# DaehwanKimLab/centrifuge

Measured on NVIDIA H100. Metric: reads/sec (100 bp SE classification), higher is better.
Workload: dtype u64

## Files before the change

centrifuge_b200/csrc/cf_logic.h:

```cpp
#ifndef CF_LOGIC_H_
#define CF_LOGIC_H_

#include <stdint.h>

#ifdef __CUDACC__
#define CFB_HD __host__ __device__ __forceinline__
#define CFB_HDN __host__ __device__
#else
#define CFB_HD inline
#define CFB_HDN inline
#endif

namespace cfb {

static const uint64_t kOff = 0xffffffffffffffffull;
static const uint64_t kUnk = 0xfffffffffffffffeull;
static const uint32_t kBwNone = 0xffffffffu;

struct IndexView {
	const uint64_t* sides;
	const uint64_t* ftab;
	const uint64_t* eftab;
	const uint16_t* sample16;
	const uint32_t* sample32;
	const uint64_t* brow;
	const uint32_t* bseq;
	const uint32_t* bbits;
	const uint64_t* seq_taxid;
	const int32_t*  seq_path;
	const uint64_t* paths;
	const uint8_t*  seq_excluded;
	const uint64_t* host_taxids;
	const uint64_t* rank16;
	const uint64_t* ftab2;
	const uint16_t* rtab16;
	const uint32_t* rtab32;
	const uint64_t* ftabk;
	const uint64_t* walk8;
	uint64_t walk8_rows;
	int32_t  ftabd_chars;
	uint64_t len, zoff, zside, fchr[4], last_boundary, num_sides;
	uint32_t zoffc, n_boundaries, n_seqs, n_host;
	int32_t  off_rate, ftab_chars, bshift, ftabk_chars;
};

struct Params {
	uint32_t khits, min_hitlen, ihits, increment;
	uint32_t tree_traverse, class_rank_slot;
};

struct HitRec { uint64_t top, bot; uint32_t bwoff, len; };

static const uint64_t kRowMask = (1ull << 40) - 1ull, kRowStart = 1ull << 63, kRowSameTs = 1ull << 58;

struct Counters {
	unsigned long long units, partial_searches, ftab_probes, sides_search, walk_steps, rows_resolved, lf_steps, ext_searches;
	unsigned long long req_rank16, req_ftab2, req_ftabk, req_walk8, req_ftabd;
};

CFB_HD int popc64(uint64_t x) {
#ifdef __CUDA_ARCH__
	return __popcll(x);
#else
	return __builtin_popcountll(x);
#endif
}

CFB_HD uint64_t match2(uint64_t w, int c) {
	uint64_t y = ~(w ^ ((uint64_t)c * 0x5555555555555555ull));
	return y & (y >> 1) & 0x5555555555555555ull;
}

CFB_HD int bwt_char(const IndexView& v, uint64_t row) {
#ifdef __CUDA_ARCH__
	if(v.rank16) {
		const uint64_t* e = v.rank16 + (row >> 6) * 8;
		const uint32_t o = (uint32_t)(row & 63);
		return (int)(((e[3] >> o) & 1ull) * 1 + ((e[5] >> o) & 1ull) * 2 + ((e[7] >> o) & 1ull) * 3);
	}
#endif
	uint64_t s = row / 384; uint32_t off = (uint32_t)(row - s * 384);
	return (int)((v.sides[s * 16 + (off >> 5)] >> ((off & 31) * 2)) & 3);
}

CFB_HD uint64_t lf_scalar(const IndexView& v, uint64_t row, int c) {
#ifdef __CUDA_ARCH__
	if(v.rank16) {
		const uint64_t* e = v.rank16 + ((row >> 6) * 4 + (uint64_t)c) * 2;
		return v.fchr[c] + (e[0] & 0x7fffffffffffffffull) + (uint64_t)popc64(e[1] & (((uint64_t)1 << (row & 63)) - 1));
	}
#endif
	uint64_t s = row / 384; uint32_t off = (uint32_t)(row - s * 384);
	const uint64_t* w = v.sides + s * 16;
	uint32_t full = off >> 5, rem = off & 31;
	uint64_t n = 0;
	for(uint32_t k = 0; k < full; k++) n += (uint64_t)popc64(match2(w[k], c));
	if(rem) n += (uint64_t)popc64(match2(w[full], c) & (((uint64_t)1 << (2 * rem)) - 1));
	if(c == 0 && s == v.zside && v.zoffc < off) n--;
	return v.fchr[c] + w[12 + c] + n;
}

CFB_HD int seq_at(const uint8_t* fw, uint32_t len, int strand, uint32_t j) {
	if(strand == 0) return fw[j];
	int c = fw[len - 1 - j];
	return c > 3 ? 4 : 3 - c;
}

CFB_HD uint64_t ftab_hi(const IndexView& v, uint64_t e) { return e <= v.len ? e : v.eftab[(e ^ kOff) * 2 + 1]; }
CFB_HD uint64_t ftab_lo(const IndexView& v, uint64_t e) { return e <= v.len ? e : v.eftab[(e ^ kOff) * 2]; }

// ... 479 lines not shown
```

centrifuge_b200/csrc/cfb200.cu:

```cuda
#include "../../include/cfb200.h"
#include "cf_index.h"
#include "cf_kernels.cuh"

#include <algorithm>
#include <atomic>
#include <mutex>
#include <thread>
#include <fcntl.h>
#include <unistd.h>
#include <cstdarg>
#include <cstdio>
#include <cstring>
#include <set>
#include <string>
#include <vector>

using namespace cfb;

enum { M_DONE = 0, M_FTAB = 1, M_LF = 2, M_NEED = 3, M_FTABK = 4 };

struct SearchArgs {
	IndexView v; Params p; BatchView b;
	HitRec* hits; uint32_t* nhits; uint32_t cap;
	unsigned long long* task_ctr64; uint32_t ntasks, chunk;
// ... 179 lines not shown
		}
		y = 0;
		for(int e = 0; e < 64; e++) if(dv[e] == 0) y |= 1ull << e;
		for(uint32_t e = 0; e < 64; e++) if(ftabk_death(y, e) != dv[e]) { y = ~0ull; break; }
	}
	const uint64_t w = bot - top;
	out[fk] = make_ulonglong2(top | ((w < kFtabkWide ? w : kFtabkWide) << 40), y);
}

template <int RW> struct ReadRegs {
	uint64_t rw[RW]; uint32_t nw[RW];
	__device__ __forceinline__ void load(const uint64_t* pk, const uint32_t* nm, uint32_t W) {
		#pragma unroll
		for(int k = 0; k < RW; k++) { rw[k] = (uint32_t)k < W ? __ldg(pk + k) : 0ull; nw[k] = (uint32_t)k < W ? __ldg(nm + k) : 0u; }
	}
	__device__ __forceinline__ uint64_t word(uint32_t k) const {
		uint64_t v = 0;
		#pragma unroll
		for(int q = 0; q < RW; q++) if((uint32_t)q == k) v = rw[q];
		return v;
	}
	__device__ __forceinline__ uint32_t nword(uint32_t k) const {
		uint32_t v = 0;
		#pragma unroll
		for(int q = 0; q < RW; q++) if((uint32_t)q == k) v = nw[q];
		return v;
	}
	__device__ __forceinline__ int base(uint32_t p) const {
		const uint32_t k = p >> 5, sh = p & 31;
		return ((nword(k) >> sh) & 1u) ? 4 : (int)((word(k) >> (2 * sh)) & 3);
	}
	__device__ __forceinline__ void window(uint32_t p, uint64_t& win, uint32_t& nwin) const {
		const uint32_t k = p >> 5, sh = p & 31;
		win = shr64(word(k), 2 * sh) | shl64(word(k + 1), 64 - 2 * sh);
		nwin = (uint32_t)(((uint64_t)nword(k) | ((uint64_t)nword(k + 1) << 32)) >> sh);
	}
};

template <int COUNT, int RW>
__global__ void __launch_bounds__(kSearchThreads) k_search_t(const SearchArgs a) {
	const ulonglong2* r16 = reinterpret_cast<const ulonglong2*>(a.v.rank16);
	const ulonglong2* ftab2 = reinterpret_cast<const ulonglong2*>(a.v.ftab2);
	const ulonglong2* ftabk = reinterpret_cast<const ulonglong2*>(a.v.ftabk);
	const uint32_t fk = (COUNT == 1 || !a.v.ftabk) ? 0u : (uint32_t)a.v.ftabk_chars;
	const uint32_t fc = (uint32_t)a.v.ftab_chars;
	const unsigned long long* w8 = COUNT == 1 ? nullptr : reinterpret_cast<const unsigned long long*>(a.v.walk8);
	const uint32_t fd = (fk == 0 || a.p.min_hitlen < (uint32_t)a.v.ftabd_chars) ? 0u : (uint32_t)a.v.ftabd_chars;
	ReadRegs<RW> rd;
	uint64_t top = 0, bot = 0, fi = 0;
	uint32_t rlen = 0, tid = 0, cur = 0, dep = 0, offset = 0, nh = 0, nt = 0, slow_until = 0, fail_w = 0, fail_at = 0xffffffffu;
	bool nolong = true;
	int mode = M_NEED;
	unsigned long long c_ps = 0, c_ft = 0, c_sides = 0, c_lf = 0;
	unsigned long long q_r16 = 0, q_f2 = 0, q_fk = 0, q_w8 = 0;
	WarpPool pool; pool.base = pool.end = 0;
	bool more = true;

	auto emit = [&](uint64_t t, uint64_t b, uint32_t off, uint32_t len) {
		if(a.keep_short || len >= kLongLen) {
			if(nh < a.cap) { HitRec* h = a.hits + (size_t)tid * a.cap + nh; h->top = t; h->bot = b; h->bwoff = off; h->len = len; }
			else atomicExch(a.overflow, 1u);
			nh++;
		}
		nt++;
		if(len >= a.p.min_hitlen) nolong = false;
	};
	auto after_hit = [&](uint32_t hlen) -> bool {
		bool done = cur >= rlen;
		if(!done) { if(hlen > a.p.increment) cur += 1; if(cur + a.p.min_hitlen >= rlen) done = true; }
		if(done) { a.nhits[tid] = nh_pack(nh, nt, nolong); mode = M_NEED; return false; }
		return true;
	};
	auto start_search = [&]() {
		for(;;) {
			if(COUNT == 1) c_ps++;
			offset = cur;
			if(rlen - cur < fc) { emit(kOff, kOff, offset, rlen - offset); a.nhits[tid] = nh_pack(nh, nt, nolong); mode = M_NEED; return; }
			uint64_t win; uint32_t nwin; rd.window(cur, win, nwin);
			const uint32_t nbits = nwin & ((1u << fc) - 1u);
			if(nbits) {
				const uint32_t hl = (uint32_t)__ffs(nbits);
				cur += hl;
				emit(kOff, kOff, offset, hl);
				if(after_hit(hl)) continue; else return;
			}
			if(fk && rlen - cur >= fk && !(nwin & ((1u << fk) - 1u))) {
				fi = win & ((1ull << (2 * fk)) - 1ull);
				if(fd && rlen - cur >= fd && !(nwin & ((1u << fd) - 1u))) fi |= (64ull | ((win >> (2 * fk)) & 63ull)) << (2 * fk);
				mode = M_FTABK;
				return;
			}
			fi = win & ((1ull << (2 * fc)) - 1ull);
			mode = M_FTAB;
			return;
		}
	};
	auto hit_and_restart = [&]() {
		const uint32_t hl = dep - offset;
		emit(top, bot, offset, hl);
		cur = dep;
		if(after_hit(hl)) start_search();
	};

	for(;;) {
		{
			const bool want = mode == M_NEED;
			if(more) {
				unsigned long long t = 0;
				const bool got = pool_take(pool, want, a.task_ctr64, (unsigned long long)a.ntasks, a.chunk, t);
				if(want) {
					if(got) {
						tid = (uint32_t)t;
						const uint32_t per = 2u * (uint32_t)a.b.n_mates;
						const uint32_t unit = tid / per, rem = tid - unit * per;
						const int mate = (int)(rem >> 1);
						const uint8_t fl = a.b.flags ? a.b.flags[unit] : 3;
						nh = 0; nt = 0; rlen = a.b.len[mate][unit];
						if(!((fl >> mate) & 1) || rlen == 0) a.nhits[tid] = 0;
						else { rd.load(a.pk + (size_t)tid * a.W, a.nm + (size_t)tid * a.W, a.W); cur = 0; slow_until = 0; fail_w = 0; fail_at = 0xffffffffu; nolong = true; start_search(); }
					} else mode = M_DONE;
				}
				if(__any_sync(0xffffffffu, want && !got)) more = false;
			} else if(want) mode = M_DONE;
		}
		if(!__any_sync(0xffffffffu, mode != M_DONE)) break;
		int c = 4;
		const bool lf = mode == M_LF;
		bool range = false, jump = false, known_fail = false;
		const void* p0 = nullptr; const void* p1 = nullptr; uint32_t sub = 0;
		if(mode == M_FTAB) { p0 = ftab2 + fi; if(COUNT == 2) q_f2++; }
		else if(mode == M_FTABK) { p0 = ftabk + (fi & ((1ull << (2 * fk)) - 1ull)); if(COUNT == 2) q_fk++; }
		else if(lf) {
			c = rd.base(dep);
			if(c <= 3) {
				range = (bot - top) != 1;
				const uint64_t width = bot - top;
				if(dep == fail_at && !range) known_fail = true;
				else if(w8 && width <= (uint64_t)a.jump_w && (dep >= slow_until || width < (uint64_t)fail_w) && rlen - dep >= 8 && bot <= a.v.walk8_rows) {
					jump = true; p0 = w8 + (top & ~1ull); sub = (uint32_t)(top & 1); if(COUNT == 2) q_w8++;
					if(range) { const uint64_t last = bot - 1; sub |= (uint32_t)(last & 1) << 1; if((last & ~1ull) != (top & ~1ull)) { p1 = w8 + (last & ~1ull); if(COUNT == 2) q_w8++; } }
				} else {
					p0 = r16 + (top >> 6) * 4 + c;
					if(COUNT == 2) q_r16++;
					if(range && (bot >> 6) != (top >> 6)) { p1 = r16 + (bot >> 6) * 4 + c; if(COUNT == 2) q_r16++; }
				}
			}
		}
		ulonglong2 e = make_ulonglong2(0, 0), bq;
		asm volatile("{\n\t.reg .pred p;\n\tsetp.ne.u64 p, %2, 0;\n\t@p ld.global.nc.v2.u64 {%0, %1}, [%2];\n\t}" : "+l"(e.x), "+l"(e.y) : "l"(p0));
		bq = e;
		asm volatile("{\n\t.reg .pred p;\n\tsetp.ne.u64 p, %2, 0;\n\t@p ld.global.nc.v2.u64 {%0, %1}, [%2];\n\t}" : "+l"(bq.x), "+l"(bq.y) : "l"(p1));
		const ulonglong2 tq = e;
		if(mode == M_FTABK) {
			const uint32_t ext = (uint32_t)(fi >> (2 * fk));
			const uint32_t dv = ext ? ftabk_death(e.y, ext & 63u) : 0u;
			const uint64_t width = e.x >> 40;
			if(dv) {
				const uint32_t hl = fk + dv - 1u;
				emit(kUnk, kUnk, offset, hl);
				cur += hl;
				if(after_hit(hl)) start_search();
			} else if(width != 0 && width != kFtabkWide) {
				top = e.x & kRowMask; bot = top + width; dep = cur + fk;
				if(dep < rlen) mode = M_LF; else hit_and_restart();
			} else { fi &= (1ull << (2 * fc)) - 1ull; mode = M_FTAB; }
		} else if(mode == M_FTAB) {
			if(COUNT == 1) c_ft++;
			top = e.x; bot = e.y;
			dep = cur + fc;
			if(bot <= top) {
				const uint32_t hl = dep - offset;
				emit(kOff, kOff, offset, hl);
				cur = dep;
				if(after_hit(hl)) start_search();
			} else if(dep < rlen) mode = M_LF;
			else hit_and_restart();
		} else if(jump) {
			uint64_t win; uint32_t nwin; rd.window(dep, win, nwin);
			const uint64_t w = (sub & 1u) ? e.y : e.x;
			const uint64_t wl = (sub & 2u) ? bq.y : bq.x;
			const uint64_t width = bot - top;
			if((w >> 56) == 8 && !(nwin & 0xffu) && !(((w >> 40) ^ win) & 0xffffull)
			   && (width == 1 || ((wl >> 40) == (w >> 40) && (wl & kWalkRowMask) - (w & kWalkRowMask) == width - 1))) {
				top = w & kWalkRowMask; bot = top + width; dep += 8;
				if(dep >= rlen) hit_and_restart();
			} else {
				slow_until = dep + 8; fail_w = (uint32_t)width;
				if(width == 1) {
					const uint32_t diff = (uint32_t)(((w >> 40) ^ win) & 0xffffull), nb = nwin & 0xffu, nv = (uint32_t)(w >> 56) & 0xffu;
					uint32_t good = diff ? (uint32_t)(__ffs(diff) - 1) >> 1 : 8u;
					if(nb) good = min(good, (uint32_t)(__ffs(nb) - 1));
					good = min(good, nv);
					fail_at = good < 8u ? dep + good : 0xffffffffu;
				}
			}
		} else if(lf) {
			bool fail = c > 3 || known_fail;
			uint64_t t = 0, b = 0;
			if(!fail) {
				const uint32_t oT = (uint32_t)(top & 63), oB = (uint32_t)(bot & 63);
				t = a.v.fchr[c] + (tq.x & kOccMask) + (uint64_t)__popcll(tq.y & ((1ull << oT) - 1ull));
				if(range) b = a.v.fchr[c] + (bq.x & kOccMask) + (uint64_t)__popcll(bq.y & ((1ull << oB) - 1ull));
				else {
					if(!((tq.y >> oT) & 1ull)) fail = true;
					b = t + 1;
				}
				if(b <= t) fail = true;
				if(COUNT == 1) {
					uint64_t sT; uint32_t offT; row_locus(top, sT, offT);
					const bool same_side = !range || (bot - top) < (uint64_t)(384 - offT);
					c_lf += range ? 2 : 1; c_sides += same_side ? 1 : 2;
				}
			}
			if(fail) hit_and_restart();
			else { top = t; bot = b; dep++; if(dep >= rlen) hit_and_restart(); }
		}
	}
	if(COUNT == 1 && a.ctr) {
		atomicAdd(&a.ctr->partial_searches, c_ps); atomicAdd(&a.ctr->ftab_probes, c_ft);
		atomicAdd(&a.ctr->sides_search, c_sides); atomicAdd(&a.ctr->lf_steps, c_lf);
	}
	if(COUNT == 2 && a.ctr) {
		atomicAdd(&a.ctr->req_rank16, q_r16); atomicAdd(&a.ctr->req_ftab2, q_f2); atomicAdd(&a.ctr->req_ftabk, q_fk); atomicAdd(&a.ctr->req_walk8, q_w8);
	}
}

struct UnitArgs {
	IndexView v; Params p; BatchView b;
	HitRec* hits; uint32_t* nhits; uint32_t cap;
	uint32_t* nrows;
	uint64_t* row_off;
	unsigned long long* row_total;
	uint64_t* rows; uint32_t* ids; uint64_t rows_cap;
	Entry* entries; TaxCnt* tcs; OutRec* recs_sparse; uint32_t* nout;
	unsigned int* overflow;
	Counters* ctr;
	HitRec* regen; uint32_t* regen_n; unsigned long long* regen_ctr; uint64_t regen_slots; uint32_t full_cap; uint32_t keep_short;
};

__device__ uint32_t search_strand_dev(const IndexView& v, const Params& p, const uint8_t* fw, uint32_t len, int strand, HitRec* hits, uint32_t cap) {
	const ulonglong2* r16 = reinterpret_cast<const ulonglong2*>(v.rank16);
	const ulonglong2* ftab2 = reinterpret_cast<const ulonglong2*>(v.ftab2);
	const ulonglong2* ftabk = reinterpret_cast<const ulonglong2*>(v.ftabk);
	const uint32_t fc = (uint32_t)v.ftab_chars, fk = v.ftabk ? (uint32_t)v.ftabk_chars : 0u;
	auto base = [&](uint32_t d) -> int { return seq_at(fw, len, strand, len - 1 - d); };
	uint32_t cur = 0, n = 0;
	if(len == 0) return 0;
	for(;;) {
		HitRec h; h.bwoff = cur; uint32_t new_cur; bool done = false;
		const uint32_t offset = cur;
		if(len - cur < fc) { h.top = h.bot = kOff; h.len = len - offset; new_cur = len; done = true; }
		else {
			uint32_t firstn = 0xffffffffu; uint64_t fi = 0;
			const uint32_t span = (fk && len - cur >= fk) ? fk : fc;
			for(uint32_t i = 0; i < span; i++) { const int c = base(cur + i); if(c > 3) { firstn = i; break; } fi |= (uint64_t)c << (2 * i); }
			if(firstn < fc) { new_cur = cur + firstn + 1; h.top = h.bot = kOff; h.len = new_cur - offset; done = new_cur >= len; }
			else {
				uint64_t top = 0, bot = 0; uint32_t dep = 0; bool have = false;
				if(span == fk && fk > fc && firstn == 0xffffffffu) {
					const uint64_t x = __ldg(&ftabk[fi].x), width = x >> 40;
					if(width != 0 && width != kFtabkWide) { top = x & kRowMask; bot = top + width; dep = cur + fk; have = true; }
				}
				if(!have) { const ulonglong2 e = __ldg(ftab2 + (fi & ((1ull << (2 * fc)) - 1ull))); top = e.x; bot = e.y; dep = cur + fc; }
				if(bot <= top) { h.top = h.bot = kOff; h.len = dep - offset; new_cur = dep; done = dep >= len; }
				else {
					while(dep < len) {
						const int c = base(dep);
						if(c > 3) break;
						if(bot - top == 1) {
							if(v.walk8 && top < v.walk8_rows && len - dep >= 8) {
								const uint64_t e = __ldg(v.walk8 + top);
								bool ok = (e >> 56) == 8;
								for(uint32_t j = 0; ok && j < 8; j++) ok = base(dep + j) == (int)((e >> (40 + 2 * j)) & 3);
								if(ok) { top = e & kWalkRowMask; bot = top + 1; dep += 8; continue; }
							}
							const ulonglong2 e = __ldg(r16 + (top >> 6) * 4 + c);
							if(!((e.y >> (top & 63)) & 1ull)) break;
							top = v.fchr[c] + (e.x & kOccMask) + (uint64_t)__popcll(e.y & ((1ull << (top & 63)) - 1ull)); bot = top + 1; dep++;
						} else {
							const ulonglong2 et = __ldg(r16 + (top >> 6) * 4 + c);
							const ulonglong2 eb = (bot >> 6) == (top >> 6) ? et : __ldg(r16 + (bot >> 6) * 4 + c);
							const uint64_t t = v.fchr[c] + (et.x & kOccMask) + (uint64_t)__popcll(et.y & ((1ull << (top & 63)) - 1ull));
							const uint64_t b = v.fchr[c] + (eb.x & kOccMask) + (uint64_t)__popcll(eb.y & ((1ull << (bot & 63)) - 1ull));
							if(b <= t) break;
							top = t; bot = b; dep++;
						}
					}
					h.top = top; h.bot = bot; h.len = dep - offset; new_cur = dep; done = dep >= len;
				}
			}
		}
		if(n < cap) hits[n] = h;
		n++;
		cur = new_cur;
		if(done) break;
		if(h.len > p.increment) cur += 1;
		if(cur + p.min_hitlen >= len) break;
	}
	return n;
}

static const uint32_t kWindowLen = 320;
template <int COUNT>
__global__ void __launch_bounds__(kSearchThreads) k_search_long(const SearchArgs a) {
	const uint32_t per = 2u * (uint32_t)a.b.n_mates;
	Counters local; memset(&local, 0, sizeof local);
	for(uint32_t tid = blockIdx.x * blockDim.x + threadIdx.x; tid < a.ntasks; tid += gridDim.x * blockDim.x) {
		const uint32_t unit = tid / per, rem = tid - unit * per;
		const int mate = (int)(rem >> 1), strand = (int)(rem & 1);
		const uint8_t fl = a.b.flags ? a.b.flags[unit] : 3;
		const uint32_t len = a.b.len[mate][unit];
		if(!((fl >> mate) & 1) || len == 0) { a.nhits[tid] = 0; continue; }
		const uint8_t* fw = a.b.bases + a.b.off[mate][unit];
		HitRec* hits = a.hits + (size_t)tid * a.cap;
		const uint32_t n = COUNT == 1 ? search_strand_scalar(a.v, a.p, fw, len, strand, hits, a.cap, &local)
		                              : search_strand_dev(a.v, a.p, fw, len, strand, hits, a.cap);
		if(n > a.cap) atomicExch(a.overflow, 1u);
		a.nhits[tid] = nh_pack(min(n, a.cap), n, false);
	}
	if(COUNT == 1 && a.ctr) {
		atomicAdd(&a.ctr->partial_searches, local.partial_searches); atomicAdd(&a.ctr->ftab_probes, local.ftab_probes);
		atomicAdd(&a.ctr->sides_search, local.sides_search); atomicAdd(&a.ctr->lf_steps, local.lf_steps);
	}
}

typedef void (*SearchKernel)(const SearchArgs);
static SearchKernel search_kernel(uint32_t maxlen, int count) {
// ... 205 lines not shown
	uint64_t idx = 0, row = 0;
	int mode = R_NEED;
	unsigned long long c_walk = 0, c_rows = 0;
	WarpPool pool; pool.base = pool.end = 0;
	bool more = true;
	auto put = [&](uint32_t v) { if(IDENT && a.ids16) a.ids16[idx] = (uint16_t)v; else a.ids[idx] = v; };
	auto settle = [&](uint64_t r) -> int {
		if(r == a.v.zoff) { if(gl == 0) put(0); return R_NEED; }
		if((r & lowmask) == 0) return R_SAMPLE;
		return R_WALK;
	};
	for(;;) {
		{
			const bool want = mode == R_NEED;
			if(more) {
				unsigned long long t = 0;
				bool got = pool_take(pool, want && gl == 0, a.task_ctr, (unsigned long long)n, a.chunk, t);
				t = __shfl_sync(0xffffffffu, t, gbase); got = __shfl_sync(0xffffffffu, (int)got, gbase) != 0;
				if(want) {
					if(got) { idx = t; row = IDENT ? idx : (a.rows[idx] & kRowMask); if(COUNT && gl == 0) c_rows++; mode = settle(row); }
					else mode = R_DONE;
				}
				if(__any_sync(0xffffffffu, want && !got)) more = false;
			} else if(want) mode = R_DONE;
		}
		if(!__any_sync(0xffffffffu, mode != R_DONE)) break;
		ulonglong2 e = make_ulonglong2(0, 0); uint32_t samp = 0;
		if(mode == R_WALK) e = __ldg(r16 + (row >> 6) * 4 + gl);
		else if(mode == R_SAMPLE && gl == 0) samp = a.v.sample32 ? __ldg(a.v.sample32 + (row >> a.v.off_rate)) : (uint32_t)__ldg(a.v.sample16 + (row >> a.v.off_rate));
		if(mode == R_SAMPLE) { if(gl == 0) put(samp); mode = R_NEED; }
		else if(mode == R_WALK) {
			const uint32_t off = (uint32_t)(row & 63);
			const unsigned flagged = __shfl_sync(gmask, (unsigned)(e.x >> 63), gbase);
			bool found = false;
			if(flagged && a.v.last_boundary > 0 && row <= a.v.last_boundary) {
				uint32_t lo = 0, hi = a.v.n_boundaries;
				while(lo < hi) { const uint32_t mid = (lo + hi) >> 1; if(a.v.brow[mid] < row) lo = mid + 1; else hi = mid; }
				if(lo < a.v.n_boundaries && a.v.brow[lo] == row) { found = true; if(gl == 0) put(a.v.sample32 ? a.v.bseq[lo] : (uint32_t)(uint16_t)a.v.bseq[lo]); }
			}
			if(found) mode = R_NEED;
			else {
				const uint64_t mine = a.v.fchr[gl] + (e.x & kOccMask) + (uint64_t)__popcll(e.y & ((1ull << off) - 1ull));
				const unsigned who = (__ballot_sync(gmask, (e.y >> off) & 1ull) >> gbase) & 0xFu;
				const int src = __ffs(who) - 1;
				row = __shfl_sync(gmask, mine, gbase + (src < 0 ? 0 : src));
				if(COUNT && gl == 0) c_walk++;
				mode = settle(row);
			}
		}
	}
	if(COUNT && gl == 0 && a.ctr) { atomicAdd(&a.ctr->walk_steps, c_walk); atomicAdd(&a.ctr->rows_resolved, c_rows); }
}

__global__ void __launch_bounds__(kSearchThreads) k_build_walk8(IndexView v, uint64_t nrows, uint64_t* out) {
	const unsigned lane = threadIdx.x & 31, gl = lane & 3, gbase = lane & 28, gmask = 0xFu << gbase;
	const ulonglong2* r16 = reinterpret_cast<const ulonglong2*>(v.rank16);
	const uint64_t ngroups = (uint64_t)gridDim.x * (kSearchThreads / 4);
	const uint64_t per = (nrows + ngroups - 1) / ngroups;
	const uint64_t g = (uint64_t)blockIdx.x * (kSearchThreads / 4) + (threadIdx.x >> 2);
	for(uint64_t idx = g * per; idx < min(nrows, (g + 1) * per); idx++) {
		uint64_t row = idx, chars = 0; uint32_t nv = 0;
		for(; nv < 8; nv++) {
			if(row == v.zoff) break;
			const ulonglong2 e = __ldg(r16 + (row >> 6) * 4 + gl);
			const uint32_t off = (uint32_t)(row & 63);
			const uint64_t mine = v.fchr[gl] + (e.x & kOccMask) + (uint64_t)__popcll(e.y & ((1ull << off) - 1ull));
			const unsigned who = (__ballot_sync(gmask, (e.y >> off) & 1ull) >> gbase) & 0xFu;
			const int src = __ffs(who) - 1;
			if(src < 0) break;
			chars |= (uint64_t)src << (2 * nv);
			row = __shfl_sync(gmask, mine, gbase + src);
		}
		if(gl == 0) out[idx] = (row & kWalkRowMask) | (chars << 40) | ((uint64_t)nv << 56);
	}
}

__global__ void __launch_bounds__(256) k_lookup(const ResolveArgs a) {
	uint64_t n = *a.total; if(n > a.rows_cap) return;
	const uint64_t i = (uint64_t)blockIdx.x * blockDim.x + threadIdx.x;
	const uint64_t stride = (uint64_t)gridDim.x * blockDim.x;
	for(uint64_t k = i; k < n; k += stride) { const uint64_t r = a.rows[k] & kRowMask; a.ids[k] = a.v.rtab32 ? __ldg(a.v.rtab32 + r) : (uint32_t)__ldg(a.v.rtab16 + r); }
}

__global__ void __launch_bounds__(128) k_compact(uint32_t n_units, const uint64_t* row_off, const uint64_t* out_off,
                                                 const OutRec* sparse, OutRec* dense, uint32_t* rec_off32, uint64_t dense_cap, unsigned int* overflow) {
	const uint32_t unit = blockIdx.x * blockDim.x + threadIdx.x;
	if(unit > n_units) return;
	if(unit == n_units) { rec_off32[unit] = (uint32_t)out_off[unit]; return; }
	const uint64_t o = out_off[unit], n = out_off[unit + 1] - o;
	rec_off32[unit] = (uint32_t)o;
	if(o + n > dense_cap) { if(n) atomicExch(overflow, 3u); return; }
	const uint64_t src = row_off[unit];
	for(uint64_t i = 0; i < n; i++) dense[o + i] = sparse[src + i];
}

__global__ void k_test_lf(IndexView v, const uint64_t* rows, const uint8_t* chars, uint64_t n, uint64_t* out) {
	for(uint64_t i = (uint64_t)blockIdx.x * blockDim.x + threadIdx.x; i < n; i += (uint64_t)gridDim.x * blockDim.x) {
		const int c = chars[i] > 3 ? bwt_char(v, rows[i]) : chars[i];
		out[i] = lf_scalar(v, rows[i], c);
	}
}

static thread_local char g_err[512] = "";
static int fail(int code, const char* fmt, ...) {
	va_list ap; va_start(ap, fmt); vsnprintf(g_err, sizeof g_err, fmt, ap); va_end(ap); return code;
}
#define CK(call) do { cudaError_t e_ = (call); if(e_ != cudaSuccess) return fail(CFB_ECUDA, "%s failed: %s (%s:%d)", #call, cudaGetErrorString(e_), __FILE__, __LINE__); } while(0)

extern "C" const char* cfb_last_error(void) { return g_err; }
extern "C" const char* cfb_version(void) { return "cfb200 0.1 (sm_90a)"; }

template <class T> struct DBuf {
	T* p = nullptr; size_t cap = 0;
	cudaError_t ensure(size_t n) {
		if(n <= cap) return cudaSuccess;
		if(p) cudaFree(p);
		p = nullptr; cap = 0;
		size_t want = n + n / 8 + 16;
		cudaError_t e = cudaMalloc((void**)&p, want * sizeof(T));
		if(e == cudaSuccess) cap = want;
		return e;
	}
	void release() { if(p) cudaFree(p); p = nullptr; cap = 0; }
};
template <class T> struct HBuf {
	T* p = nullptr; size_t cap = 0;
// ... 106 lines not shown
			uint64_t* f2 = nullptr; const uint64_t nf = h.ftab_len - 1;
			CKX(cudaMalloc((void**)&f2, nf * 16));
			ix->dptrs.push_back(f2); ix->device_bytes += nf * 16;
			k_build_ftab2<<<(unsigned)((nf + 255) / 256), 256>>>(v, nf, f2);
			CKX(cudaDeviceSynchronize());
			v.rank16 = r16; v.ftab2 = f2;
			ix->tables.rank16_bytes = (nb + 1) * 64; ix->tables.ftab2_bytes = nf * 16;
			cudaFree((void*)v.sides);
			ix->dptrs.erase(std::find(ix->dptrs.begin(), ix->dptrs.end(), (void*)v.sides));
			ix->device_bytes -= h.num_sides * h.side_sz; v.sides = nullptr;
			size_t free_b = 0, total_b = 0; cudaMemGetInfo(&free_b, &total_b);
			double head_gb = 12.0; { const char* e = getenv("CFB_HBM_HEADROOM_GB"); if(e) head_gb = atof(e); }
			const uint64_t headroom = std::min<uint64_t>((uint64_t)(head_gb * 1073741824.0), free_b / 2);
			auto budget = [&]() -> uint64_t { size_t f = 0, t = 0; cudaMemGetInfo(&f, &t); return f > headroom ? f - headroom : 0; };
			{
				const char* ed = getenv("CFB_FTABD");
				const bool death = !(ed && ed[0] == '0');
				int K = 0;
				{ const char* e = getenv("CFB_FTABK"); if(e) K = atoi(e); else { K = h.ftab_chars; while(K < 15 && (4ull << (2 * K)) <= h.len / 4) K++; } }
				while(K > h.ftab_chars && (16ull << (2 * K)) > budget() / 2) K--;
				if(K <= h.ftab_chars || K > 16) K = death ? h.ftab_chars : 0;
				const uint64_t nk = K ? 1ull << (2 * K) : 0;
				if(K && h.len + 1 < (1ull << 40) && nk * 16 <= budget()) {
					ulonglong2* fk = nullptr;
					CKX(cudaMalloc((void**)&fk, nk * 16));
					ix->dptrs.push_back(fk); ix->device_bytes += nk * 16;
					k_build_ftabk<<<(unsigned)((nk + 127) / 128), 128>>>(v, K, nk, death, fk);
					CKX(cudaDeviceSynchronize());
					v.ftabk = (const uint64_t*)fk; v.ftabk_chars = K; v.ftabd_chars = death ? K + 3 : 0;
					ix->tables.ftabk_bytes = nk * 16; ix->tables.ftabk_chars = K; ix->tables.ftabd_chars = v.ftabd_chars;
				}
			}
			{
				const char* e = (flags & CFB_LOAD_NO_RESOLVE_TABLE) ? "0" : getenv("CFB_RESOLVE_TABLE");
				const uint64_t nrows = h.len + 1, esz = h.wide_sample ? 4 : 2;
				if(!(e && e[0] == '0') && nrows * esz + 16 <= budget()) {
					void* tab = nullptr; unsigned long long* sc = nullptr;
					CKX(cudaMalloc(&tab, nrows * esz + 16)); CKX(cudaMalloc((void**)&sc, 16));
					ix->dptrs.push_back(tab); ix->device_bytes += nrows * esz;
					const unsigned long long init[2] = {0ull, (unsigned long long)nrows};
					CKX(cudaMemcpy(sc, init, 16, cudaMemcpyHostToDevice));
					ResolveArgs ra; ra.v = v; ra.rows = nullptr; ra.ids = h.wide_sample ? (uint32_t*)tab : nullptr; ra.ids16 = h.wide_sample ? nullptr : (uint16_t*)tab;
					ra.total = (const uint64_t*)(sc + 1); ra.rows_cap = nrows; ra.task_ctr = sc; ra.chunk = 256; ra.ctr = nullptr;
					int occ = 1; cudaOccupancyMaxActiveBlocksPerMultiprocessor(&occ, k_resolve_c<false, true>, kSearchThreads, 0);
					k_resolve_c<false, true><<<prop.multiProcessorCount * std::max(occ, 1), kSearchThreads>>>(ra);
					CKX(cudaDeviceSynchronize());
					cudaFree(sc);
					if(h.wide_sample) v.rtab32 = (const uint32_t*)tab; else v.rtab16 = (const uint16_t*)tab;
					ix->tables.resolve_table_bytes = nrows * esz; ix->tables.resolve_entry_bytes = (int32_t)esz;
				}
			}
			{
				const char* e = (flags & CFB_LOAD_NO_WALK8) ? "0" : getenv("CFB_WALK8");
				const uint64_t nrows = h.len + 1;
				uint64_t cover = std::min<uint64_t>(nrows, budget() / 8);
				{ const char* f = getenv("CFB_WALK8_ROWS"); if(f) cover = std::min<uint64_t>(nrows, strtoull(f, NULL, 10)); }
				if(!(e && e[0] == '0') && nrows < (1ull << 40) && cover >= nrows / 8 && cover > 0) {
					void* tab = nullptr;
					CKX(cudaMalloc(&tab, cover * 8 + 16));
					ix->dptrs.push_back(tab); ix->device_bytes += cover * 8;
					int occ = 1; cudaOccupancyMaxActiveBlocksPerMultiprocessor(&occ, k_build_walk8, kSearchThreads, 0);
					k_build_walk8<<<prop.multiProcessorCount * std::max(occ, 1) * 4, kSearchThreads>>>(v, cover, (uint64_t*)tab);
					CKX(cudaDeviceSynchronize());
					v.walk8 = (const uint64_t*)tab; v.walk8_rows = cover;
					ix->tables.walk8_bytes = cover * 8; ix->tables.walk8_rows = cover;
				}
			}
		}
		{ size_t fb = 0, tb = 0; cudaMemGetInfo(&fb, &tb); ix->tables.total_bytes = ix->device_bytes; ix->tables.free_bytes_after_load = fb; }
		std::vector<uint8_t>().swap(ix->h.sides);
	}
	*out = ix;
	return CFB_OK;
}
#undef CKX
extern "C" int cfb_index_load(const char* basename, int device, cfb_index** out) { return cfb_index_load_ex(basename, device, 0u, out); }
extern "C" void cfb_index_free(cfb_index* ix) {
	if(!ix) return;
	if(ix->device >= 0) { cudaSetDevice(ix->device); for(size_t i = 0; i < ix->dptrs.size(); i++) cudaFree(ix->dptrs[i]); }
	delete ix;
}
extern "C" int cfb_index_get_info(const cfb_index* ix, cfb_index_info* o) {
	if(!ix || !o) return fail(CFB_EINVAL, "null argument");
	const HostIndex& h = ix->h;
	o->len = h.len; o->num_sides = h.num_sides; o->n_seqs = h.seq_taxid.size(); o->n_tax_nodes = h.nodes.size();
	o->n_boundaries = h.brow.size(); o->line_rate = h.line_rate; o->off_rate = h.off_rate; o->ftab_chars = h.ftab_chars;
	o->sample_bytes = h.wide_sample ? 4 : 2; o->compressed = h.compressed ? 1 : 0; o->device = ix->device; o->device_bytes = ix->device_bytes;
	return CFB_OK;
}
extern "C" int cfb_index_get_tables(const cfb_index* ix, cfb_index_tables* o) {
	if(!ix || !o) return fail(CFB_EINVAL, "null argument");
	*o = ix->tables;
	return CFB_OK;
}
extern "C" const char* cfb_index_seq_name(const cfb_index* ix, uint32_t s) { return (ix && s < ix->h.seq_name.size()) ? ix->h.seq_name[s].c_str() : NULL; }
extern "C" uint64_t cfb_index_seq_taxid(const cfb_index* ix, uint32_t s) { return (ix && s < ix->h.seq_taxid.size()) ? ix->h.seq_taxid[s] : 0; }
extern "C" int cfb_index_tax_node(const cfb_index* ix, uint64_t taxid, uint64_t* parent, int* rank, int* leaf) {
	const TaxNode* n = ix ? ix->h.find_node(taxid) : NULL;
	if(!n) return 0;
	if(parent) *parent = n->parent; if(rank) *rank = n->rank; if(leaf) *leaf = n->leaf;
	return 1;
}
extern "C" const cfb::HostIndex* cfb_index_host(const cfb_index* ix) { return ix ? &ix->h : NULL; }
extern "C" int cfb_index_node_taxids(const cfb_index* ix, uint64_t* out, uint64_t cap) {
	if(!ix || !out || cap < ix->h.nodes.size()) return fail(CFB_EINVAL, "cfb_index_node_taxids: buffer too small");
	for(size_t i = 0; i < ix->h.nodes.size(); i++) out[i] = ix->h.nodes[i].taxid;
	return CFB_OK;
}
extern "C" void cfb_params_default(cfb_params* p) {
	if(!p) return;
	memset(p, 0, sizeof *p); p->khits = 5; p->min_hitlen = 22; p->tree_traverse = 1; p->class_rank_slot = 0;
}

static const int kSlots = 17;

struct Slot {
	cudaStream_t st = nullptr;
	cudaEvent_t ev[6] = {nullptr, nullptr, nullptr, nullptr, nullptr, nullptr};
// ... 24 lines not shown

struct cfb_dbatch { int slot; uint64_t n_units; };
struct TextCtx;
static void text_release(cfb_ctx*);
static void comm_release(cfb_ctx*);

struct CountsCtx {
	bool ready = false;
	std::vector<uint64_t> h_taxid; DBuf<uint64_t> d_taxid; uint32_t n = 0;
	DBuf<unsigned long long> total, global; bool reduced = false;
	void release() { d_taxid.release(); total.release(); global.release(); }
};

struct cfb_ctx {
	const cfb_index* ix = nullptr;
	IndexView view; Params prm;
	DBuf<uint8_t> d_excl; DBuf<uint64_t> d_host;
	Slot slots[kSlots];
	Counters* d_ctr = nullptr; int count = 0;
	uint64_t launches = 0;
	int resolve_blocks = 0;
	cfb_dbatch resident; bool resident_used = false;
	double rec_ratio = 2.0;
	uint64_t rows_cap0 = 0;
	TextCtx* text = nullptr;
	CountsCtx cnt; bool fold_records = false;
	uint32_t jump_w = 4; bool keep_short = false;
	uint64_t regen_lists = 0, regen_tasks = 0;
	uint64_t regen_slots0 = 0;
	void* comm = nullptr; int comm_rank = 0, comm_size = 1; cudaStream_t comm_st = nullptr;
};

static void expand_taxids(const HostIndex& h, const uint64_t* ids, uint64_t n, std::set<uint64_t>& out) {
	if(n == 0 || !ids) return;
	for(size_t i = 0; i < h.nodes.size(); i++) {
		uint64_t t = h.nodes[i].taxid;
		for(;;) {
			bool found = false;
			for(uint64_t k = 0; k < n; k++) if(ids[k] == t) { found = true; break; }
			if(found) { out.insert(h.nodes[i].taxid); break; }
			const TaxNode* nd = h.find_node(t);
			if(!nd || nd->parent == t) break;
			t = nd->parent;
		}
	}
}

extern "C" void cfb_ctx_destroy(cfb_ctx* c) {
	if(!c) return;
	if(c->ix && c->ix->device >= 0) cudaSetDevice(c->ix->device);
	if(getenv("CFB_REGEN_STATS") && c->regen_tasks)
		fprintf(stderr, "[cfb] strand lists regenerated by k_prep: %llu of %llu (%.3f %%)\n", (unsigned long long)c->regen_lists,
		        (unsigned long long)c->regen_tasks, 100.0 * (double)c->regen_lists / (double)c->regen_tasks);
	text_release(c);
	comm_release(c);
	c->cnt.release();
	for(int i = 0; i < kSlots; i++) c->slots[i].release();
	c->d_excl.release(); c->d_host.release();
	if(c->d_ctr) cudaFree(c->d_ctr);
	delete c;
}

extern "C" int cfb_ctx_create(const cfb_index* ix, const cfb_params* p, cfb_ctx** out) {
	if(!ix || !p || !out) return fail(CFB_EINVAL, "cfb_ctx_create: null argument");
	if(ix->device < 0) return fail(CFB_ENODEV, "index was loaded host-only; classification needs a CUDA device (no CPU fallback)");
	if(p->khits < 1) return fail(CFB_EINVAL, "khits must be >= 1");
	CK(cudaSetDevice(ix->device));
	cfb_ctx* c = new cfb_ctx();
	c->ix = ix; c->view = ix->view;
	const HostIndex& h = ix->h;
	Params& q = c->prm;
	q.khits = (uint32_t)p->khits;
	q.min_hitlen = (uint32_t)(p->min_hitlen < 15 ? 15 : p->min_hitlen);
	q.ihits = (uint32_t)std::max(p->khits, 5) * (h.compressed ? 4u : 40u);
	q.increment = (2 * q.min_hitlen <= 33) ? 10 : (2 * q.min_hitlen - 33);
	q.tree_traverse = p->tree_traverse ? 1 : 0;
	q.class_rank_slot = (uint32_t)(p->class_rank_slot & 0xff);
	std::set<uint64_t> host, excl;
	expand_taxids(h, p->host_taxids, p->n_host_taxids, host);
	expand_taxids(h, p->excluded_taxids, p->n_excluded_taxids, excl);
	#define CKC(call) do { cudaError_t e_ = (call); if(e_ != cudaSuccess) { cfb_ctx_destroy(c); return fail(CFB_ECUDA, "%s failed: %s", #call, cudaGetErrorString(e_)); } } while(0)
	if(!excl.empty()) {
		std::vector<uint8_t> fl(h.seq_taxid.size(), 0);
		for(size_t i = 0; i < fl.size(); i++) fl[i] = excl.count(h.seq_taxid[i]) ? 1 : 0;
		CKC(c->d_excl.ensure(fl.size())); CKC(cudaMemcpy(c->d_excl.p, fl.data(), fl.size(), cudaMemcpyHostToDevice));
		c->view.seq_excluded = c->d_excl.p;
	}
	if(!host.empty()) {
		std::vector<uint64_t> hv(host.begin(), host.end());
		CKC(c->d_host.ensure(hv.size())); CKC(cudaMemcpy(c->d_host.p, hv.data(), hv.size() * 8, cudaMemcpyHostToDevice));
		c->view.host_taxids = c->d_host.p; c->view.n_host = (uint32_t)hv.size();
	}
	for(int i = 0; i < kSlots; i++) {
		CKC(cudaStreamCreateWithFlags(&c->slots[i].st, cudaStreamNonBlocking));
		for(int e = 0; e < 6; e++) CKC(cudaEventCreate(&c->slots[i].ev[e]));
		CKC(c->slots[i].scal.ensure(8)); CKC(c->slots[i].h_scal.ensure(8));
	}
	CKC(cudaMalloc((void**)&c->d_ctr, sizeof(Counters))); CKC(cudaMemset(c->d_ctr, 0, sizeof(Counters)));
	{
		const char* e = getenv("CFB_L2_FETCH"); const size_t g = e ? (size_t)atoi(e) : 32;
		if(g == 32 || g == 64 || g == 128) cudaDeviceSetLimit(cudaLimitMaxL2FetchGranularity, g);
		const char* pe = getenv("CFB_L2_PERSIST");
		if(pe && pe[0] == '1') {
			cudaDeviceSetLimit(cudaLimitPersistingL2CacheSize, 16u << 20);
			for(int i = 0; i < kSlots; i++) {
				cudaStreamAttrValue av; memset(&av, 0, sizeof av);
// ... 496 lines not shown
```

Baseline: 258.0 million.

## Sample walk8 table per 64-row block and support variable-length jumps

Replaces the walk8 jump table, which covered only a prefix of BWT rows, with a table that stores the first S rows of every 64-row rank block. Entries hold a variable jump length k (up to 8) that ends on a sampled row, so a chain of jumps can stay inside the table. The search and resolve kernels index the table by block and offset and accept k-step jumps instead of requiring exactly 8. This spreads table coverage across the whole BWT under the same memory budget, at the cost of shorter jumps and a fallback to rank16 lookups for unsampled offsets. It also adds a single-row rank16 request counter and a stats printout behind an environment variable.

```diff
diff --git a/centrifuge_b200/csrc/cf_logic.h b/centrifuge_b200/csrc/cf_logic.h
--- a/centrifuge_b200/csrc/cf_logic.h
+++ b/centrifuge_b200/csrc/cf_logic.h
@@ -37,7 +37,7 @@
 	const uint32_t* rtab32;
 	const uint64_t* ftabk;
 	const uint64_t* walk8;
-	uint64_t walk8_rows;
+	uint64_t walk8_s;
 	int32_t  ftabd_chars;
 	uint64_t len, zoff, zside, fchr[4], last_boundary, num_sides;
 	uint32_t zoffc, n_boundaries, n_seqs, n_host;
@@ -56,6 +56,7 @@
 struct Counters {
 	unsigned long long units, partial_searches, ftab_probes, sides_search, walk_steps, rows_resolved, lf_steps, ext_searches;
 	unsigned long long req_rank16, req_ftab2, req_ftabk, req_walk8, req_ftabd;
+	unsigned long long req_rank16_single;
 };
 
 CFB_HD int popc64(uint64_t x) {
diff --git a/centrifuge_b200/csrc/cfb200.cu b/centrifuge_b200/csrc/cfb200.cu
--- a/centrifuge_b200/csrc/cfb200.cu
+++ b/centrifuge_b200/csrc/cfb200.cu
@@ -255,7 +255,7 @@
 	bool nolong = true;
 	int mode = M_NEED;
 	unsigned long long c_ps = 0, c_ft = 0, c_sides = 0, c_lf = 0;
-	unsigned long long q_r16 = 0, q_f2 = 0, q_fk = 0, q_w8 = 0;
+	unsigned long long q_r16 = 0, q_r16s = 0, q_f2 = 0, q_fk = 0, q_w8 = 0;
 	WarpPool pool; pool.base = pool.end = 0;
 	bool more = true;
 
@@ -339,12 +339,14 @@
 				range = (bot - top) != 1;
 				const uint64_t width = bot - top;
 				if(dep == fail_at && !range) known_fail = true;
-				else if(w8 && width <= (uint64_t)a.jump_w && (dep >= slow_until || width < (uint64_t)fail_w) && rlen - dep >= 8 && bot <= a.v.walk8_rows) {
-					jump = true; p0 = w8 + (top & ~1ull); sub = (uint32_t)(top & 1); if(COUNT == 2) q_w8++;
-					if(range) { const uint64_t last = bot - 1; sub |= (uint32_t)(last & 1) << 1; if((last & ~1ull) != (top & ~1ull)) { p1 = w8 + (last & ~1ull); if(COUNT == 2) q_w8++; } }
+				else if(w8 && width <= (uint64_t)a.jump_w && (dep >= slow_until || width < (uint64_t)fail_w) && rlen - dep >= 8
+				        && (top & 63) < a.v.walk8_s && ((bot - 1) & 63) < a.v.walk8_s) {
+					const uint64_t it = (top >> 6) * a.v.walk8_s + (top & 63);
+					jump = true; p0 = w8 + (it & ~1ull); sub = (uint32_t)(it & 1); if(COUNT == 2) q_w8++;
+					if(range) { const uint64_t il = ((bot - 1) >> 6) * a.v.walk8_s + ((bot - 1) & 63); sub |= (uint32_t)(il & 1) << 1; if((il & ~1ull) != (it & ~1ull)) { p1 = w8 + (il & ~1ull); if(COUNT == 2) q_w8++; } }
 				} else {
 					p0 = r16 + (top >> 6) * 4 + c;
-					if(COUNT == 2) q_r16++;
+					if(COUNT == 2) { q_r16++; if(!range) q_r16s++; }
 					if(range && (bot >> 6) != (top >> 6)) { p1 = r16 + (bot >> 6) * 4 + c; if(COUNT == 2) q_r16++; }
 				}
 			}
@@ -383,18 +385,17 @@
 			const uint64_t w = (sub & 1u) ? e.y : e.x;
 			const uint64_t wl = (sub & 2u) ? bq.y : bq.x;
 			const uint64_t width = bot - top;
-			if((w >> 56) == 8 && !(nwin & 0xffu) && !(((w >> 40) ^ win) & 0xffffull)
-			   && (width == 1 || ((wl >> 40) == (w >> 40) && (wl & kWalkRowMask) - (w & kWalkRowMask) == width - 1))) {
-				top = w & kWalkRowMask; bot = top + width; dep += 8;
+			const uint32_t k = (uint32_t)(w >> 56);
+			const uint32_t diff = (uint32_t)(((w >> 40) ^ win) & ((1ull << (2 * k)) - 1ull)), nb = nwin & ((1u << k) - 1u);
+			if(k && !diff && !nb && (width == 1 || ((wl >> 40) == (w >> 40) && (wl & kWalkRowMask) - (w & kWalkRowMask) == width - 1))) {
+				top = w & kWalkRowMask; bot = top + width; dep += k;
 				if(dep >= rlen) hit_and_restart();
 			} else {
 				slow_until = dep + 8; fail_w = (uint32_t)width;
 				if(width == 1) {
-					const uint32_t diff = (uint32_t)(((w >> 40) ^ win) & 0xffffull), nb = nwin & 0xffu, nv = (uint32_t)(w >> 56) & 0xffu;
-					uint32_t good = diff ? (uint32_t)(__ffs(diff) - 1) >> 1 : 8u;
+					uint32_t good = diff ? (uint32_t)(__ffs(diff) - 1) >> 1 : k;
 					if(nb) good = min(good, (uint32_t)(__ffs(nb) - 1));
-					good = min(good, nv);
-					fail_at = good < 8u ? dep + good : 0xffffffffu;
+					fail_at = good < k || k == 0 ? dep + good : 0xffffffffu;
 				}
 			}
 		} else if(lf) {
@@ -425,6 +426,7 @@
 	}
 	if(COUNT == 2 && a.ctr) {
 		atomicAdd(&a.ctr->req_rank16, q_r16); atomicAdd(&a.ctr->req_ftab2, q_f2); atomicAdd(&a.ctr->req_ftabk, q_fk); atomicAdd(&a.ctr->req_walk8, q_w8);
+		atomicAdd(&a.ctr->req_rank16_single, q_r16s);
 	}
 }
 
@@ -471,11 +473,12 @@
 						const int c = base(dep);
 						if(c > 3) break;
 						if(bot - top == 1) {
-							if(v.walk8 && top < v.walk8_rows && len - dep >= 8) {
-								const uint64_t e = __ldg(v.walk8 + top);
-								bool ok = (e >> 56) == 8;
-								for(uint32_t j = 0; ok && j < 8; j++) ok = base(dep + j) == (int)((e >> (40 + 2 * j)) & 3);
-								if(ok) { top = e & kWalkRowMask; bot = top + 1; dep += 8; continue; }
+							if(v.walk8 && (top & 63) < v.walk8_s && len - dep >= 8) {
+								const uint64_t e = __ldg(v.walk8 + (top >> 6) * v.walk8_s + (top & 63));
+								const uint32_t k = (uint32_t)(e >> 56);
+								bool ok = k > 0;
+								for(uint32_t j = 0; ok && j < k; j++) ok = base(dep + j) == (int)((e >> (40 + 2 * j)) & 3);
+								if(ok) { top = e & kWalkRowMask; bot = top + 1; dep += k; continue; }
 							}
 							const ulonglong2 e = __ldg(r16 + (top >> 6) * 4 + c);
 							if(!((e.y >> (top & 63)) & 1ull)) break;
@@ -787,14 +790,17 @@
 	if(COUNT && gl == 0 && a.ctr) { atomicAdd(&a.ctr->walk_steps, c_walk); atomicAdd(&a.ctr->rows_resolved, c_rows); }
 }
 
-__global__ void __launch_bounds__(kSearchThreads) k_build_walk8(IndexView v, uint64_t nrows, uint64_t* out) {
+__global__ void __launch_bounds__(kSearchThreads) k_build_walk8(IndexView v, uint64_t nent, uint64_t* out) {
 	const unsigned lane = threadIdx.x & 31, gl = lane & 3, gbase = lane & 28, gmask = 0xFu << gbase;
 	const ulonglong2* r16 = reinterpret_cast<const ulonglong2*>(v.rank16);
+	const uint64_t S = v.walk8_s;
 	const uint64_t ngroups = (uint64_t)gridDim.x * (kSearchThreads / 4);
-	const uint64_t per = (nrows + ngroups - 1) / ngroups;
+	const uint64_t per = (nent + ngroups - 1) / ngroups;
 	const uint64_t g = (uint64_t)blockIdx.x * (kSearchThreads / 4) + (threadIdx.x >> 2);
-	for(uint64_t idx = g * per; idx < min(nrows, (g + 1) * per); idx++) {
-		uint64_t row = idx, chars = 0; uint32_t nv = 0;
+	for(uint64_t idx = g * per; idx < min(nent, (g + 1) * per); idx++) {
+		const uint64_t r0 = (idx / S) * 64 + idx % S;
+		if(r0 > v.len) { if(gl == 0) out[idx] = 0; continue; }
+		uint64_t row = r0, chars = 0, lrow = 0; uint32_t nv = 0, lk = 0;
 		for(; nv < 8; nv++) {
 			if(row == v.zoff) break;
 			const ulonglong2 e = __ldg(r16 + (row >> 6) * 4 + gl);
@@ -805,8 +811,10 @@
 			if(src < 0) break;
 			chars |= (uint64_t)src << (2 * nv);
 			row = __shfl_sync(gmask, mine, gbase + src);
-		}
-		if(gl == 0) out[idx] = (row & kWalkRowMask) | (chars << 40) | ((uint64_t)nv << 56);
+			if((row & 63) < S) { lrow = row; lk = nv + 1; }
+		}
+		if(lk == 0) { lrow = row; lk = nv; }
+		if(gl == 0) out[idx] = (lrow & kWalkRowMask) | ((chars & ((1ull << (2 * lk)) - 1ull)) << 40) | ((uint64_t)lk << 56);
 	}
 }
 
@@ -1019,18 +1027,20 @@
 			}
 			{
 				const char* e = (flags & CFB_LOAD_NO_WALK8) ? "0" : getenv("CFB_WALK8");
-				const uint64_t nrows = h.len + 1;
-				uint64_t cover = std::min<uint64_t>(nrows, budget() / 8);
-				{ const char* f = getenv("CFB_WALK8_ROWS"); if(f) cover = std::min<uint64_t>(nrows, strtoull(f, NULL, 10)); }
-				if(!(e && e[0] == '0') && nrows < (1ull << 40) && cover >= nrows / 8 && cover > 0) {
+				const uint64_t nrows = h.len + 1, nblk = (nrows + 63) / 64;
+				uint64_t S = std::min<uint64_t>(64, budget() / 8 / nblk);
+				{ const char* f = getenv("CFB_WALK8_ROWS"); if(f) S = std::min<uint64_t>(S, std::max<uint64_t>(1, strtoull(f, NULL, 10) / nblk)); }
+				if(!(e && e[0] == '0') && nrows < (1ull << 40) && S >= 8) {
+					const uint64_t nent = nblk * S;
 					void* tab = nullptr;
-					CKX(cudaMalloc(&tab, cover * 8 + 16));
-					ix->dptrs.push_back(tab); ix->device_bytes += cover * 8;
+					CKX(cudaMalloc(&tab, nent * 8 + 16));
+					ix->dptrs.push_back(tab); ix->device_bytes += nent * 8;
+					v.walk8_s = S;
 					int occ = 1; cudaOccupancyMaxActiveBlocksPerMultiprocessor(&occ, k_build_walk8, kSearchThreads, 0);
-					k_build_walk8<<<prop.multiProcessorCount * std::max(occ, 1) * 4, kSearchThreads>>>(v, cover, (uint64_t*)tab);
+					k_build_walk8<<<prop.multiProcessorCount * std::max(occ, 1) * 4, kSearchThreads>>>(v, nent, (uint64_t*)tab);
 					CKX(cudaDeviceSynchronize());
-					v.walk8 = (const uint64_t*)tab; v.walk8_rows = cover;
-					ix->tables.walk8_bytes = cover * 8; ix->tables.walk8_rows = cover;
+					v.walk8 = (const uint64_t*)tab;
+					ix->tables.walk8_bytes = nent * 8; ix->tables.walk8_rows = (nrows / 64) * S + std::min<uint64_t>(S, nrows % 64);
 				}
 			}
 		}
@@ -1161,6 +1171,14 @@
 	if(getenv("CFB_REGEN_STATS") && c->regen_tasks)
 		fprintf(stderr, "[cfb] strand lists regenerated by k_prep: %llu of %llu (%.3f %%)\n", (unsigned long long)c->regen_lists,
 		        (unsigned long long)c->regen_tasks, 100.0 * (double)c->regen_lists / (double)c->regen_tasks);
+	if(getenv("CFB_REQ_STATS") && c->count == 2 && c->d_ctr) {
+		Counters h; memset(&h, 0, sizeof h);
+		if(cudaMemcpy(&h, c->d_ctr, sizeof h, cudaMemcpyDeviceToHost) == cudaSuccess && h.units) {
+			const double u = (double)h.units;
+			fprintf(stderr, "[cfb] search requests per unit (%llu units): rank16 %.2f = single row %.2f + range %.2f; K-mer %.2f, 10-mer %.2f, walk8 %.2f\n",
+			        h.units, h.req_rank16 / u, h.req_rank16_single / u, (h.req_rank16 - h.req_rank16_single) / u, h.req_ftabk / u, h.req_ftab2 / u, h.req_walk8 / u);
+		}
+	}
 	text_release(c);
 	comm_release(c);
 	c->cnt.release();
```

Measured after the change: 263.2 million, median of 6. +2.0%, better.
